# jeff-regier/Celeste.jl

Measured on AMD Instinct MI355X. Metric: sources/sec (ELBO value+gradient+Hessian+KL per target source), higher is better.
Workload: dtype f64; 1 GPU; BASELINE.json configs[2]: synthetic 2048x1489x5 SDSS-size field, 2000 star+galaxy sources, fp64, Sa=1 with value-only neighbours, psf_K=2; gather_backend=none, neighbor_links_rank0=3526

## Files before the change

### celeste.jl_amd/csrc/celeste_abi.hip

```cpp
#include <hip/hip_runtime.h>
#include <algorithm>
#include <atomic>
#include <cmath>
#include <cstdio>
#include <cstdlib>
#include <cstring>
#include <mutex>
#include <unordered_map>
#include <vector>

#include "elbo_kernels.h"
#include "optim_kernels.h"
#include "fused_kernels.h"
#include "host_tables.h"
#include "value_union.h"

struct celeste_group;

#define EVAL_FUSED_MAX 32

#define HIP_TRY(expr)                                                                    \
    do {                                                                                 \
        hipError_t e__ = (expr);                                                         \
        if (e__ != hipSuccess) {                                                         \
// ... 87 lines not shown
    std::vector<void *> plane_allocs;
    DevImage *d_images = nullptr;
    std::atomic<int> refs{1};
};

static void images_release(celeste_images *im) {
    if (!im || im->refs.fetch_sub(1) != 1) return;
    (void)hipSetDevice(im->device);
    for (void *p : im->plane_allocs) (void)hipFree(p);
    if (im->d_images) (void)hipFree(im->d_images);
    delete im;
}

struct celeste_ctx {
    int device = 0;
    celeste_images *imgs = nullptr;
    hipStream_t stream = nullptr;
    hipStream_t copy_stream = nullptr;
    bool copy_stream_checked = false;
    int N = 0, S = 0, K = 0, NC = 0, n_stamps = 0;
    int chunk_px = 256, CH = 1;
    int max_npx = 0;
    std::vector<DevPatch> h_patches;
    std::vector<int64_t> h_nbr_off;
    std::vector<int32_t> h_nbr_idx;
    DevImage *d_images = nullptr;
    DevPatch *d_patches = nullptr;
    double *d_coefs = nullptr;
    float *d_coefs_f = nullptr;
    uint8_t *d_bitmaps = nullptr;
    int64_t *d_nbr_off = nullptr;
    int32_t *d_nbr_idx = nullptr;
    PriorDev *d_prior = nullptr;
    SrcImg *d_srcimg = nullptr;
    Comp *d_comps = nullptr;
    SrcGeo *d_geo = nullptr;
    int64_t *d_val_off = nullptr;
    double2 *d_val = nullptr;
    int32_t *d_needed = nullptr;
    int32_t stamp = 0;
    std::vector<int32_t> h_vis_off, h_vis_img, h_vis_src;
    int32_t *d_vis_off = nullptr, *d_vis_img = nullptr, *d_vis_src = nullptr;
    int4 *d_value_items = nullptr;
    int4 *d_vitems_src = nullptr;
    int32_t *d_vitem_off = nullptr;
    std::vector<int32_t> h_vitem_off;
    std::vector<int32_t> h_vitem_tgt;
    std::vector<ValueUnionLink> h_vitem_link;
    int64_t n_value_items = 0;
    std::vector<struct celeste_targets *> lists;
    int32_t *d_prep_mark = nullptr;
    double *d_lg_sum = nullptr;
    int64_t *d_nv_base = nullptr;
    int32_t *d_nbr_vis = nullptr;
    int2 *d_items = nullptr;
    size_t items_cap = 0;
    std::vector<int32_t> h_src_chunks;
    std::vector<int64_t> h_top_chunks;
    int max_src_chunks = 0;
    int32_t *d_work = nullptr, *d_work_blk = nullptr, *d_work_total = nullptr;
    size_t work_cap = 0, work_blk_cap = 0;
    int M = 1;
    bool dense = false;
    int64_t V = 0;
    std::vector<int64_t> h_tile_off;
    int64_t *d_tile_off = nullptr;
    int64_t n_tiles = 0;
    int sum_tiles = 4, RCH = 1;
    double *d_rec = nullptr;
    double *d_acc_split = nullptr;
    size_t acc_split_cap = 0;
    double *d_acc = nullptr;
    size_t acc_cap = 0;
    int32_t *d_rec_off = nullptr;
    size_t rec_off_cap = 0;
    double *d_vp = nullptr;
    int32_t *d_targets = nullptr;
    double *d_v = nullptr, *d_d = nullptr, *d_h = nullptr;
    int64_t *d_cnt = nullptr;
    int32_t *d_status = nullptr;
    size_t stage_cap = 0;
    double *p_vp = nullptr;
    int32_t *p_targets = nullptr, *p_status = nullptr;
    double *p_v = nullptr, *p_d = nullptr, *p_h = nullptr;
    int64_t *p_cnt = nullptr;
    size_t pin_cap = 0;
    double *d_small_in = nullptr, *p_small_in = nullptr, *d_small_out = nullptr, *p_small_out = nullptr;
    static const int MAX_PARTS = 8;
    hipEvent_t part_done[MAX_PARTS] = {}, part_copied[MAX_PARTS] = {};
    struct OptBuffers {
        size_t cap = 0;
        double *d_vp = nullptr, *d_v = nullptr, *d_d = nullptr, *d_h = nullptr, *d_H = nullptr, *d_T = nullptr, *d_S = nullptr, *d_pos = nullptr;
        int32_t *d_targets = nullptr, *d_act[2] = {nullptr, nullptr}, *d_evt[2] = {nullptr, nullptr}, *d_count = nullptr,
                *d_st = nullptr;
        void *d_state = nullptr;
        static const int RING = 4;
        double *h_vp = nullptr;
        void *h_state = nullptr;
        int32_t *h_count = nullptr;
        hipEvent_t ev[RING] = {};
    } opt;
    struct FusedBuffers {
        size_t cap_t = 0, cap_rec = 0, cap_q = 0, cap_saved = 0;
        bool arrivals_dirty = true;
        int4 *d_chunk_desc = nullptr;
        int2 *d_tgt_rec = nullptr;
// ... 294 lines not shown
            if (device >= 0 && device < 16) consts_ready[device] = true;
        }
    }
    CTX_TRY(dev_upload<SrcImg>(&c->d_srcimg, nullptr, (size_t)c->V));
    CTX_TRY(dev_upload<Comp>(&c->d_comps, nullptr, (size_t)c->V * c->NC));
    CTX_TRY(dev_upload<SrcGeo>(&c->d_geo, nullptr, (size_t)c->S));
    {
        std::vector<int64_t> voff(c->h_patches.size());
        int64_t tot = 0;
        for (size_t q = 0; q < c->h_patches.size(); ++q) { voff[q] = tot; tot += (int64_t)c->h_patches[q].H2 * c->h_patches[q].W2; }
        CTX_TRY(dev_upload(&c->d_val_off, voff.data(), voff.size()));
        CTX_TRY(dev_upload<double2>(&c->d_val, nullptr, (size_t)tot));
        CTX_TRY(dev_upload<int32_t>(&c->d_needed, nullptr, (size_t)c->S));
        if (hipMemset(c->d_needed, 0, (size_t)c->S * sizeof(int32_t)) != hipSuccess) { celeste_ctx_destroy(c); return CELESTE_ERR_HIP; }
    }

    CTX_TRY(dev_upload(&c->d_vis_off, c->h_vis_off.data(), c->h_vis_off.size()));
    CTX_TRY(dev_upload(&c->d_vis_img, c->h_vis_img.data(), c->h_vis_img.size()));
    CTX_TRY(dev_upload(&c->d_vis_src, c->h_vis_src.data(), c->h_vis_src.size()));
    CTX_TRY(dev_upload<double>(&c->d_lg_sum, nullptr, (size_t)c->V));
    if (c->V > 0)
        hipLaunchKernelGGL(patch_lgamma_kernel, dim3((unsigned)c->V), dim3(256), 0, nullptr, c->d_images, c->d_patches,
                           c->d_vis_img, c->d_bitmaps, c->d_lg_sum);
    const char *env_chunk = getenv("CELESTE_CHUNK_PX");
    if (env_chunk && atoi(env_chunk) >= 64) c->chunk_px = (atoi(env_chunk) + 63) / 64 * 64;
    c->CH = c->max_npx > 0 ? (c->max_npx + c->chunk_px - 1) / c->chunk_px : 1;
    c->h_src_chunks.assign((size_t)c->S, 0);
    for (int s = 0; s < c->S; ++s) {
        for (int v = c->h_vis_off[s]; v < c->h_vis_off[s + 1]; ++v) {
            const DevPatch &q = c->h_patches[v];
            c->h_src_chunks[s] += (q.H2 * q.W2 + c->chunk_px - 1) / c->chunk_px;
        }
        c->max_src_chunks = std::max(c->max_src_chunks, c->h_src_chunks[s]);
    }
    auto hv = [c](int s, int n) -> int64_t {
        if (c->dense) return (int64_t)s * c->N + n;
        const int32_t *b = c->h_vis_img.data() + c->h_vis_off[s], *e = c->h_vis_img.data() + c->h_vis_off[s + 1];
        const int32_t *it = std::lower_bound(b, e, n);
        return it != e && *it == n ? (int64_t)(it - c->h_vis_img.data()) : -1;
    };
    if (!c->dense) {
        std::vector<int64_t> base((size_t)c->S + 1, 0);
        for (int s = 0; s < c->S; ++s)
            base[s + 1] = base[s] + (int64_t)(c->h_vis_off[s + 1] - c->h_vis_off[s]) * (c->h_nbr_off[s + 1] - c->h_nbr_off[s]);
        std::vector<int32_t> nv((size_t)base[c->S]);
        for (int s = 0; s < c->S; ++s) {
            const int64_t K = c->h_nbr_off[s + 1] - c->h_nbr_off[s];
            for (int v = c->h_vis_off[s]; v < c->h_vis_off[s + 1]; ++v)
                for (int64_t q = 0; q < K; ++q)
                    nv[base[s] + (int64_t)(v - c->h_vis_off[s]) * K + q] = (int32_t)hv(c->h_nbr_idx[c->h_nbr_off[s] + q], c->h_vis_img[v]);
        }
        CTX_TRY(dev_upload(&c->d_nv_base, base.data(), base.size()));
        CTX_TRY(dev_upload(&c->d_nbr_vis, nv.data(), nv.size()));
    }
    {
        std::vector<int32_t> sorted(c->h_src_chunks);
        std::sort(sorted.begin(), sorted.end(), [](int32_t a, int32_t b) { return a > b; });
        c->h_top_chunks.assign((size_t)c->S + 1, 0);
        for (int s = 0; s < c->S; ++s) c->h_top_chunks[s + 1] = c->h_top_chunks[s] + sorted[s];
    }
    CTX_TRY(dev_upload<int32_t>(&c->d_work_total, nullptr, 1));
    {
        if (c->N > 0xffff) { celeste_ctx_destroy(c); return CELESTE_ERR_INVALID_ARG; }
        const int n_cls = c->chunk_px / 64;
        std::vector<std::vector<std::pair<int32_t, int32_t>>> by_len(n_cls);
        for (int s = 0; s < c->S; ++s)
            for (int64_t q = c->h_nbr_off[s]; q < c->h_nbr_off[s + 1]; ++q) {
                const int s2 = c->h_nbr_idx[q];
                for (int va = c->h_vis_off[s]; va < c->h_vis_off[s + 1]; ++va) {
                    const int n = c->h_vis_img[va];
                    const int64_t vb = hv(s2, n);
                    if (vb < 0) continue;
                    const DevPatch &a = c->h_patches[va], &b = c->h_patches[vb];
                    const int rh = std::min(a.off_h + a.H2, b.off_h + b.H2) - std::max(a.off_h, b.off_h);
                    const int rw = std::min(a.off_w + a.W2, b.off_w + b.W2 - 1) - std::max(a.off_w, b.off_w);
                    if (rh <= 0 || rw <= 0) continue;
                    const int npx = rh * rw, nch = (npx + c->chunk_px - 1) / c->chunk_px;
                    for (int ch = 0; ch < nch; ++ch) {
                        const int px = std::min(c->chunk_px, npx - ch * c->chunk_px);
                        by_len[n_cls - (px + 63) / 64].push_back({(int32_t)q, (int32_t)(n | (ch << 16))});
                    }
                }
            }
        std::vector<int32_t> link_src(c->h_nbr_idx.size());
        for (int s = 0; s < c->S; ++s)
            for (int64_t q = c->h_nbr_off[s]; q < c->h_nbr_off[s + 1]; ++q) link_src[q] = s;
        std::vector<int4> desc;
        for (auto &v : by_len)
            for (auto &e : v) {
                const int t = link_src[e.first], s2 = c->h_nbr_idx[e.first], n = e.second & 0xffff, ch = e.second >> 16;
                desc.push_back(make_int4((int)hv(s2, n), (int)hv(t, n), ch, t));
            }
        c->n_value_items = (int64_t)desc.size();
        c->h_vitem_tgt.resize(desc.size());
        c->h_vitem_link.resize(desc.size());
        for (size_t i = 0; i < desc.size(); ++i) { c->h_vitem_tgt[i] = desc[i].w; c->h_vitem_link[i] = {desc[i].x, desc[i].y}; }
        CTX_TRY(dev_upload(&c->d_value_items, desc.data(), desc.size()));
        c->h_vitem_off.assign((size_t)c->S + 1, 0);
        for (auto &d : desc) c->h_vitem_off[(size_t)d.w + 1]++;
        for (int s = 0; s < c->S; ++s) c->h_vitem_off[s + 1] += c->h_vitem_off[s];
        {
            std::vector<int4> by_src(desc.size());
            std::vector<int32_t> fill(c->h_vitem_off.begin(), c->h_vitem_off.end() - 1);
            for (auto &d : desc) by_src[(size_t)fill[d.w]++] = d;
            CTX_TRY(dev_upload(&c->d_vitems_src, by_src.data(), by_src.size()));
            CTX_TRY(dev_upload(&c->d_vitem_off, c->h_vitem_off.data(), c->h_vitem_off.size()));
// ... 312 lines not shown
        if (flags & CELESTE_FLAG_HESS) LAUNCH_PIXEL_M(2);
        else if (derivs) LAUNCH_PIXEL_M(1);
        else LAUNCH_PIXEL_M(0);
    }
    else if (split) LAUNCH_PIXEL(3);
    else if (flags & CELESTE_FLAG_HESS) LAUNCH_PIXEL(2);
    else if (derivs) LAUNCH_PIXEL(1);
    else LAUNCH_PIXEL_T(0, double);
#undef LAUNCH_PIXEL
#undef LAUNCH_PIXEL_M
#undef PIXEL_ARGS
#undef LAUNCH_PIXEL_T
    if (c->timing) HIP_TRY(hipEventRecord(c->ev[2], stream));
    c->ev_split = 0;
    const int lift_nt = n_targets <= 1024 ? 512 : 256;
    bool lift7 = n_targets > 4096;
    if (const char *e = getenv("CELESTE_LIFT_WAVES")) lift7 = atoi(e) == 7;
#define LAUNCH_LIFT(...) do { if (lift7) hipLaunchKernelGGL(lift_kernel<7>, __VA_ARGS__); else hipLaunchKernelGGL(lift_kernel<8>, __VA_ARGS__); } while (0)
    if (split) {
        hipLaunchKernelGGL(record_sum_kernel, dim3((unsigned)((size_t)n_targets * c->M * c->RCH)), dim3(RSUM_NT), 0,
                           stream, c->d_patches, d_targets, c->d_tile_off, reinterpret_cast<const double2 *>(c->d_rec),
                           c->d_items, c->N, c->M, c->RCH, c->sum_tiles, c->d_acc_split, nullptr, c->d_work_total);
        if (c->timing) { HIP_TRY(hipEventRecord(c->ev[4], stream)); c->ev_split = 1; }
        LAUNCH_LIFT(dim3(n_targets), dim3(lift_nt), 0, stream, d_vp, c->d_images, c->d_patches, c->d_geo,
                           c->d_nbr_off, c->d_nbr_idx, d_targets, c->d_acc_split, c->d_prior, c->d_vis_off, c->d_vis_img, c->N, c->M,
                           c->RCH, c->sum_tiles * 64, flags,
                           d_v, d_d, d_h, d_counters, d_status, d_live, d_active_rank ? nullptr : c->d_lg_sum, nullptr, d_h_pos);
    } else
    LAUNCH_LIFT(dim3(n_targets), dim3(lift_nt), 0, stream, d_vp, c->d_images, c->d_patches, c->d_geo,
                       c->d_nbr_off, c->d_nbr_idx, d_targets, c->d_acc, c->d_prior, c->d_vis_off, c->d_vis_img, c->N, c->M, CH,
                       chunk_px, flags,
                       d_v, d_d, d_h, d_counters, d_status, d_live, d_active_rank ? nullptr : c->d_lg_sum, c->d_rec_off, d_h_pos);
#undef LAUNCH_LIFT
    if (c->timing) { HIP_TRY(hipEventRecord(c->ev[3], stream)); c->ev_valid = 1; }
    HIP_TRY(hipGetLastError());
    return CELESTE_OK;
}

struct celeste_targets {
    celeste_ctx_t *ctx = nullptr;
    int32_t n = 0;
    int G = 1;
    int32_t *d_targets = nullptr;
    int32_t *d_work = nullptr, *d_work_total = nullptr, *d_rec_off = nullptr;
    int2 *d_items = nullptr;
    int32_t *d_needed = nullptr;
    int32_t *d_visits = nullptr;
    int32_t *d_vitems = nullptr;
    int4 *d_uitems = nullptr;
    int32_t *d_upx = nullptr;
    int64_t n_visits = 0, n_vitems = 0, n_uitems = 0;
    int64_t n_records = 0;
    int32_t n_work = 0;
};
static const int32_t LIST_STAMP = 1;

static void targets_free(celeste_targets *t) {
    if (!t) return;
    void *ptrs[] = {t->d_targets, t->d_work, t->d_work_total, t->d_rec_off, t->d_items, t->d_needed, t->d_visits, t->d_vitems,
                    t->d_uitems, t->d_upx};
    for (void *p : ptrs) if (p) (void)hipFree(p);
    delete t;
}

static int targets_build(celeste_ctx_t *c, const std::vector<int32_t> &tg, celeste_targets_t **out) {
    const int32_t n = (int32_t)tg.size();
    if ((size_t)n * c->M * c->CH > 0x7fffffffull) return CELESTE_ERR_INVALID_ARG;
    HIP_TRY(hipSetDevice(c->device));
    celeste_targets *t = new celeste_targets;
    t->ctx = c; t->n = n; t->G = chunk_group(n);
    int32_t *d_blk = nullptr;
    auto fail = [&](int st) { if (d_blk) (void)hipFree(d_blk); (void)hipGetLastError(); targets_free(t); return st; };
#define LIST_TRY(expr) do { if ((expr) != hipSuccess) return fail(CELESTE_ERR_HIP); } while (0)
#define LIST_ALLOC(p, bytes) do { if (hipMalloc((void **)&(p), (bytes)) != hipSuccess) return fail(CELESTE_ERR_ALLOC); } while (0)
    std::vector<char> is_tgt((size_t)c->S, 0), reads((size_t)c->S, 0);
    for (int32_t s : tg) {
        is_tgt[s] = 1; reads[s] = 1;
        for (int64_t q = c->h_nbr_off[s]; q < c->h_nbr_off[s + 1]; ++q) reads[c->h_nbr_idx[q]] = 1;
        t->n_records += c->h_src_chunks[s];
    }
    std::vector<int32_t> visits, vitems;
    for (int s = 0; s < c->S; ++s)
        if (reads[s]) for (int v = c->h_vis_off[s]; v < c->h_vis_off[s + 1]; ++v) visits.push_back(v);
    for (size_t i = 0; i < c->h_vitem_tgt.size(); ++i) if (is_tgt[c->h_vitem_tgt[i]]) vitems.push_back((int32_t)i);
    std::vector<int32_t> upx;
    std::vector<ValueUnionItem> uitems;
    {
        static_assert(sizeof(ValueUnionBox) == 4 * sizeof(int32_t) && sizeof(ValueUnionItem) == sizeof(int4), "layout");
        std::vector<ValueUnionBox> boxes(c->h_patches.size());
        for (size_t v = 0; v < boxes.size(); ++v) { const DevPatch &q = c->h_patches[v]; boxes[v] = {q.off_h, q.off_w, q.H2, q.W2}; }
        std::vector<ValueUnionLink> links;
        links.reserve(vitems.size());
        for (int32_t i : vitems) links.push_back(c->h_vitem_link[(size_t)i]);
        if (!value_union_build(boxes.data(), std::move(links), c->chunk_px, upx, uitems)) return fail(CELESTE_ERR_INVALID_ARG);
    }
    t->n_visits = (int64_t)visits.size(); t->n_vitems = (int64_t)vitems.size(); t->n_uitems = (int64_t)uitems.size();
    const int n_cand = n * c->M;
    const int n_wblk = (n_cand + WORK_NT - 1) / WORK_NT;
    const size_t n_blk = (size_t)n_wblk * (WORK_CLASSES + 1);
    LIST_ALLOC(t->d_targets, (size_t)n * sizeof(int32_t));
    LIST_ALLOC(t->d_work, std::max<size_t>((size_t)t->n_records, 1) * sizeof(int32_t));
    LIST_ALLOC(t->d_work_total, sizeof(int32_t));
    LIST_ALLOC(t->d_rec_off, (size_t)n_cand * sizeof(int32_t));
    if (!c->dense) LIST_ALLOC(t->d_items, (size_t)n_cand * sizeof(int2));
    LIST_ALLOC(t->d_needed, (size_t)c->S * sizeof(int32_t));
    LIST_ALLOC(t->d_visits, std::max<size_t>(visits.size(), 1) * sizeof(int32_t));
    LIST_ALLOC(t->d_vitems, std::max<size_t>(vitems.size(), 1) * sizeof(int32_t));
    LIST_ALLOC(t->d_uitems, std::max<size_t>(uitems.size(), 1) * sizeof(int4));
    LIST_ALLOC(t->d_upx, std::max<size_t>(upx.size(), 1) * sizeof(int32_t));
    LIST_ALLOC(d_blk, n_blk * sizeof(int32_t));
    LIST_TRY(hipMemcpy(t->d_targets, tg.data(), (size_t)n * sizeof(int32_t), hipMemcpyHostToDevice));
    if (!visits.empty()) LIST_TRY(hipMemcpy(t->d_visits, visits.data(), visits.size() * sizeof(int32_t), hipMemcpyHostToDevice));
    if (!vitems.empty()) LIST_TRY(hipMemcpy(t->d_vitems, vitems.data(), vitems.size() * sizeof(int32_t), hipMemcpyHostToDevice));
    if (!uitems.empty()) LIST_TRY(hipMemcpy(t->d_uitems, uitems.data(), uitems.size() * sizeof(int4), hipMemcpyHostToDevice));
    if (!upx.empty()) LIST_TRY(hipMemcpy(t->d_upx, upx.data(), upx.size() * sizeof(int32_t), hipMemcpyHostToDevice));
    LIST_TRY(hipMemset(t->d_needed, 0, (size_t)c->S * sizeof(int32_t)));
    const size_t setup_threads = (size_t)n * (c->dense ? 1 : c->M);
    hipLaunchKernelGGL(setup_kernel, dim3((unsigned)((setup_threads + 63) / 64)), dim3(64), 0, nullptr, (const double *)nullptr, -1,
                       (SrcGeo *)nullptr, t->d_targets, n, c->d_vis_off, c->d_vis_img, c->M, t->d_items, t->d_needed, LIST_STAMP,
                       (int32_t *)nullptr, c->d_nbr_off, c->d_nbr_idx, (const int32_t *)nullptr);
    hipLaunchKernelGGL(work_count_kernel, dim3(n_wblk), dim3(WORK_NT), 0, nullptr, t->d_targets, n_cand, c->d_patches,
                       c->d_vis_off, c->d_vis_img, c->N, c->M, c->chunk_px, t->G, (int)c->dense, d_blk, (const int32_t *)nullptr);
    hipLaunchKernelGGL(work_scan_kernel, dim3(1), dim3(1024), 0, nullptr, d_blk, (int)n_blk, t->d_work_total, n_wblk * WORK_CLASSES);
    hipLaunchKernelGGL(work_fill_kernel, dim3(n_wblk), dim3(WORK_NT), 0, nullptr, t->d_targets, n_cand, c->d_patches,
                       c->d_vis_off, c->d_vis_img, c->N, c->M, c->CH, c->chunk_px, t->G, (int)c->dense, d_blk, t->d_work,
                       (const int32_t *)nullptr, t->d_rec_off);
    LIST_TRY(hipGetLastError());
    LIST_TRY(hipMemcpy(&t->n_work, t->d_work_total, sizeof(int32_t), hipMemcpyDeviceToHost));
    LIST_TRY(hipFree(d_blk)); d_blk = nullptr;
#undef LIST_TRY
#undef LIST_ALLOC
    if (t->n_work < 0 || (int64_t)t->n_work > t->n_records) return fail(CELESTE_ERR_HIP);
    c->lists.push_back(t);
    *out = t;
    return CELESTE_OK;
}

extern "C" int celeste_targets_create(celeste_ctx_t *c, int32_t n_targets, const int32_t *targets, celeste_targets_t **out) try {
    if (!c || !out || !targets || n_targets <= 0) return CELESTE_ERR_INVALID_ARG;
    *out = nullptr;
    for (int32_t i = 0; i < n_targets; ++i) if (targets[i] < 0 || targets[i] >= c->S) return CELESTE_ERR_INVALID_ARG;
    return targets_build(c, std::vector<int32_t>(targets, targets + n_targets), out);
} ABI_CATCH

extern "C" int celeste_targets_create_device(celeste_ctx_t *c, int32_t n_targets, const int32_t *d_targets, void *stream_,
                                             celeste_targets_t **out) try {
    if (!c || !out || !d_targets || n_targets <= 0) return CELESTE_ERR_INVALID_ARG;
    *out = nullptr;
    HIP_TRY(hipSetDevice(c->device));
    std::vector<int32_t> tg((size_t)n_targets);
    HIP_TRY(hipMemcpyAsync(tg.data(), d_targets, (size_t)n_targets * sizeof(int32_t), hipMemcpyDeviceToHost, (hipStream_t)stream_));
    HIP_TRY(hipStreamSynchronize((hipStream_t)stream_));
    for (int32_t s : tg) if (s < 0 || s >= c->S) return CELESTE_ERR_INVALID_ARG;
    return targets_build(c, tg, out);
} ABI_CATCH

static void targets_release(celeste_targets_t *t) {
    celeste_ctx_t *c = t->ctx;
    auto it = std::find(c->lists.begin(), c->lists.end(), t);
    if (it != c->lists.end()) c->lists.erase(it);
    targets_free(t);
}

extern "C" void celeste_targets_destroy(celeste_targets_t *t) {
    if (!t) return;
    (void)hipSetDevice(t->ctx->device);
    (void)hipDeviceSynchronize();
    targets_release(t);
}

static int launch_prepared(celeste_ctx_t *c, const celeste_targets_t *t, const double *d_vp, uint32_t flags, double *d_v,
                           double *d_d, double *d_h, int64_t *d_counters, int32_t *d_status, void *stream_) {
    if (!c || !t || t->ctx != c) return CELESTE_ERR_INVALID_ARG;
    const int32_t n_targets = t->n;
    const char *off = getenv("CELESTE_NO_PREPARED");
    if ((off && atoi(off) != 0) || (flags & (CELESTE_FLAG_FP32 | CELESTE_FLAG_SPLIT)) ||
        want_eval_fused(flags, n_targets, true, d_d, d_h))
        return launch_eval(c, d_vp, n_targets, t->d_targets, flags, d_v, d_d, d_h, d_counters, d_status, stream_, true, nullptr,
                           t->n_records);
    if (!d_vp || !d_v || !d_status) return CELESTE_ERR_INVALID_ARG;
    if ((flags & CELESTE_FLAG_HESS) && !d_h) return CELESTE_ERR_INVALID_ARG;
    if ((flags & (CELESTE_FLAG_GRAD | CELESTE_FLAG_HESS)) && !d_d) return CELESTE_ERR_INVALID_ARG;
    hipStream_t stream = (hipStream_t)stream_;
    HIP_TRY(hipSetDevice(c->device));
    const size_t need = std::max<size_t>((size_t)t->n_records, 1) * ACC_N;
    if (need > c->acc_cap) {
        if (c->d_acc) { HIP_TRY(hipStreamSynchronize(stream)); HIP_TRY(hipFree(c->d_acc)); c->d_acc = nullptr; }
        HIP_TRY(hipMalloc((void **)&c->d_acc, need * sizeof(double)));
        c->acc_cap = need;
    }
    const int CH = c->CH, chunk_px = c->chunk_px;
    if (c->timing) HIP_TRY(hipEventRecord(c->ev[0], stream));
    const unsigned geo_blocks = (unsigned)((c->S + 63) / 64);
    hipLaunchKernelGGL(geo_prep_kernel, dim3(geo_blocks + (unsigned)t->n_visits), dim3(64), 0, stream, d_vp, c->d_images,
                       c->d_patches, c->d_vis_src, c->d_vis_img, c->K, c->d_srcimg, c->d_comps, t->d_visits, (int)geo_blocks,
                       c->S, c->d_geo);
    const char *no_union = getenv("CELESTE_NO_VALUE_UNION");
    if (!(no_union && atoi(no_union) != 0)) {
        if (t->n_uitems > 0) {
            const bool wide_items = n_targets <= VALUE_WIDE_MAX && c->chunk_px == 256 && !getenv("CELESTE_NO_WIDE_VALUE");
#define LAUNCH_UNION(WAVES)                                                                                                 \
            hipLaunchKernelGGL((value_union_kernel<WAVES>), dim3((unsigned)t->n_uitems), dim3(64 * WAVES), 0, stream,       \
                               c->d_patches, c->d_coefs, c->d_srcimg, c->d_comps, c->d_val_off, t->d_uitems, t->d_upx,      \
                               c->NC, c->d_val)
            if (wide_items) LAUNCH_UNION(4); else LAUNCH_UNION(1);
#undef LAUNCH_UNION
        }
    } else if (t->n_vitems > 0) {
        const bool wide_items = n_targets <= VALUE_WIDE_MAX && c->chunk_px == 256 && !getenv("CELESTE_NO_WIDE_VALUE");
#define LAUNCH_VALUE(WAVES)                                                                                                 \
        hipLaunchKernelGGL((value_kernel<double, WAVES>), dim3((unsigned)t->n_vitems), dim3(64 * WAVES), 0, stream,        \
                           c->d_patches, c->d_coefs, c->d_srcimg, c->d_comps, t->d_needed, LIST_STAMP, c->d_val_off,        \
                           c->d_value_items, c->NC, c->chunk_px, c->d_val, c->d_coefs_f, t->d_vitems)
        if (wide_items) LAUNCH_VALUE(4); else LAUNCH_VALUE(1);
#undef LAUNCH_VALUE
    }
    if (c->timing) HIP_TRY(hipEventRecord(c->ev[1], stream));
    const dim3 grid((unsigned)std::max<int32_t>(t->n_work, 1));
#define LAUNCH_PIXEL(MODE)                                                                                                  \
    hipLaunchKernelGGL((pixel_kernel<MODE, double>), grid, dim3(64), 0, stream, c->d_images, c->d_patches, c->d_coefs,      \
                       c->d_bitmaps, c->d_srcimg, c->d_comps, c->d_nbr_off, c->d_nbr_idx, c->d_val_off, c->d_val,           \
                       t->d_targets, c->N, c->NC, CH, chunk_px, t->G, c->d_acc, c->d_tile_off, c->d_rec,                    \
                       (const int32_t *)nullptr, t->d_items, c->M, t->d_work, t->d_work_total, c->d_nv_base, c->d_nbr_vis,  \
                       t->d_rec_off, c->d_coefs_f)
    if (flags & CELESTE_FLAG_HESS) LAUNCH_PIXEL(2);
    else if (flags & CELESTE_FLAG_GRAD) LAUNCH_PIXEL(1);
    else LAUNCH_PIXEL(0);
#undef LAUNCH_PIXEL
    if (c->timing) HIP_TRY(hipEventRecord(c->ev[2], stream));
    c->ev_split = 0;
    const int lift_nt = n_targets <= 1024 ? 512 : 256;
    bool lift7 = n_targets > 4096;
    if (const char *e = getenv("CELESTE_LIFT_WAVES")) lift7 = atoi(e) == 7;
#define LIFT_ARGS dim3(n_targets), dim3(lift_nt), 0, stream, d_vp, c->d_images, c->d_patches, c->d_geo, c->d_nbr_off,       \
                  c->d_nbr_idx, t->d_targets, c->d_acc, c->d_prior, c->d_vis_off, c->d_vis_img, c->N, c->M, CH, chunk_px,   \
                  flags, d_v, d_d, d_h, d_counters, d_status, (const int32_t *)nullptr, c->d_lg_sum, t->d_rec_off, \
                  (const int32_t *)nullptr
    if (lift7) hipLaunchKernelGGL(lift_kernel<7>, LIFT_ARGS); else hipLaunchKernelGGL(lift_kernel<8>, LIFT_ARGS);
#undef LIFT_ARGS
    if (c->timing) { HIP_TRY(hipEventRecord(c->ev[3], stream)); c->ev_valid = 1; }
    HIP_TRY(hipGetLastError());
    return CELESTE_OK;
}

extern "C" int celeste_elbo_eval_targets_device(celeste_ctx_t *c, const celeste_targets_t *t, const double *d_vp, uint32_t flags,
                                                double *d_v, double *d_d, double *d_h, int64_t *d_counters,
                                                int32_t *d_status, void *stream_) try {
    return launch_prepared(c, t, d_vp, flags, d_v, d_d, d_h, d_counters, d_status, stream_);
} ABI_CATCH

__global__ void spin_kernel(long long ticks) {
    const long long t0 = wall_clock64();
    while (wall_clock64() - t0 < ticks) __builtin_amdgcn_s_sleep(8);
}
static int pick_copy_stream(celeste_ctx_t *c) {
    if (c->copy_stream_checked) return CELESTE_OK;
    c->copy_stream_checked = true;
    if (const char *e = getenv("CELESTE_COPY_STREAM_CHECK")) if (atoi(e) == 0) return CELESTE_OK;
    const size_t bytes = 4u << 20;
    void *d_buf = nullptr, *h_buf = nullptr;
    hipEvent_t e0 = nullptr, e1 = nullptr;
    if (hipMalloc(&d_buf, bytes) != hipSuccess || hipHostMalloc(&h_buf, bytes, hipHostMallocDefault) != hipSuccess ||
        hipEventCreate(&e0) != hipSuccess || hipEventCreate(&e1) != hipSuccess) {
        (void)hipGetLastError();
        if (d_buf) (void)hipFree(d_buf);
        if (h_buf) (void)hipHostFree(h_buf);
        if (e0) (void)hipEventDestroy(e0);
        if (e1) (void)hipEventDestroy(e1);
        return CELESTE_OK;
    }
    const float spin_ms = 0.3f;
    auto measure = [&](hipStream_t s, float *ms) -> bool {
        if (hipEventRecord(e0, c->stream) != hipSuccess) return false;
        hipLaunchKernelGGL(spin_kernel, dim3(1), dim3(64), 0, c->stream, (long long)(spin_ms * 1e5));
        if (hipStreamWaitEvent(s, e0, 0) != hipSuccess || hipMemcpyAsync(h_buf, d_buf, bytes, hipMemcpyDeviceToHost, s) != hipSuccess ||
            hipEventRecord(e1, s) != hipSuccess || hipStreamSynchronize(s) != hipSuccess || hipStreamSynchronize(c->stream) != hipSuccess)
            return false;
        return hipEventElapsedTime(ms, e0, e1) == hipSuccess;
// ... 1016 lines not shown
```

### celeste.jl_amd/csrc/elbo_kernels.h

```cpp
#pragma once
#include <hip/hip_runtime.h>
#include <math.h>
#include "elbo_device.h"
#include "../../include/celeste_mi355x.h"

#ifndef CELESTE_MUTANT
#define CELESTE_MUTANT 0
#endif

__constant__ double c_eta[16];
__constant__ double c_nu[16];

__device__ inline void bvn_cov(double ab, double angle, double scale, double &x11, double &x12, double &x22) {
    double sp, cp;
    sincos(angle, &sp, &cp);
    double ab_term = ab * ab - 1.0;
    double s2 = scale * scale;
    x12 = -s2 * cp * sp * ab_term;
    x11 = s2 * (1.0 + ab_term * (sp * sp));
    x22 = s2 * (1.0 + ab_term * (cp * cp));
}

__device__ inline void brightness(const double *vs, int i, int b, double &El, double &Ell) {
    const double r = vs[6 + i], v = vs[8 + i];
    const double *cm = vs + 10 + 4 * i, *cv = vs + 18 + 4 * i;
    double l = r + 0.5 * v, ll = 2 * r + 2 * v;
    if (b >= 3) { l += cm[2] + .5 * cv[2]; ll += 2 * cm[2] + 2 * cv[2]; }
    if (b >= 4) { l += cm[3] + .5 * cv[3]; ll += 2 * cm[3] + 2 * cv[3]; }
    if (b <= 1) { l += -cm[1] + .5 * cv[1]; ll += -2 * cm[1] + 2 * cv[1]; }
    if (b <= 0) { l += -cm[0] + .5 * cv[0]; ll += -2 * cm[0] + 2 * cv[0]; }
    double e = exp(r + 0.5 * v), ee = exp(2 * r + 2 * v);
    if (b >= 3) { e *= exp(cm[2] + .5 * cv[2]); ee *= exp(2 * cm[2] + 2 * cv[2]); }
    if (b >= 4) { e *= exp(cm[3] + .5 * cv[3]); ee *= exp(2 * cm[3] + 2 * cv[3]); }
    if (b <= 1) { e *= exp(-cm[1] + .5 * cv[1]); ee *= exp(-2 * cm[1] + 2 * cv[1]); }
    if (b <= 0) { e *= exp(-cm[0] + .5 * cv[0]); ee *= exp(-2 * cm[0] + 2 * cv[0]); }
    (void)l; (void)ll;
    El = e; Ell = ee;
}

__device__ __forceinline__ void world_to_pix(const double *__restrict__ vs, const DevPatch &p, double &m1, double &m2) {
    const double d0 = vs[0] - p.wc[0], d1 = vs[1] - p.wc[1];
    m1 = p.J[0] * d0 + p.J[2] * d1 + p.pc[0];
    m2 = p.J[1] * d0 + p.J[3] * d1 + p.pc[1];
}
template <bool MOMENTS = true>
__device__ __forceinline__ void prep_visit_values(int c, const double *__restrict__ vs, const DevPatch &p, int b, int K,
                                                  SrcImg *__restrict__ si_out, Comp *__restrict__ comps_out) {
    const int NC = 14 * K;
    double m1, m2;
    world_to_pix(vs, p, m1, m2);
    double x11, x12, x22;
    bvn_cov(vs[3], vs[4], vs[5], x11, x12, x22);
    if (c < NC) {
        int i, j, k;
        if (c < 8 * K) { i = 0; k = c / 8; j = c - 8 * k; }
        else { int cc = c - 8 * K; i = 1; k = cc / 6; j = cc - 6 * k; }
// ... 1913 lines not shown
        __syncthreads();
    }
    __shared__ double tcx[(MODE == 2 || MODE == 3) && sizeof(R) == 8 ? COMPX * (14 * CEL_MAXK + 1) : 1];
    if constexpr ((MODE == 2 || MODE == 3) && sizeof(R) == 8) {
        if (lane < NC) comp_extra(tc[lane], tcx + COMPX * lane);
        __syncthreads();
    }
    PixWork<R> W;
    W.img = &images[n]; W.P = &P; W.patches = patches; W.bitmaps = bitmaps; W.nbr_idx = nbr_idx;
    W.nb0 = nbr_off[t]; W.nb1 = nbr_off[t + 1];
    W.nv = nbr_vis ? nbr_vis + nv_base[t] + (int64_t)(tn - ti * M) * (W.nb1 - W.nb0) : nullptr;
    W.val_off = val_off; W.val = val; W.active_rank = active_rank;
    W.my_rank = MULTI ? active_rank[t] : 0;
    W.N = N; W.n = n; W.NC = NC; W.v = v;
    W.si = srcimg[v];
    W.tc = tc; W.tcx = tcx;
    W.tcr = sizeof(R) == 4 ? reinterpret_cast<const CompR<R> *>(tcr_f) : reinterpret_cast<const CompR<R> *>(tc);
    W.etab = etab;
    W.tcoef = coefs + (size_t)(CELESTE_MUTANT == 3 ? 0 : P.stamp) * (CEL_COEF * CEL_COEF);
    W.tcoef_f = coefs_f + (size_t)(CELESTE_MUTANT == 3 ? 0 : P.stamp) * (CEL_COEF * CEL_COEF);
    W.tile_off = tile_off; W.rec = rec;
    __shared__ double sacc[MODE == 0 || MODE == 3 ? 1 : ACC_N * ACC_SLOTS];
    double *const slot = sacc + (lane & (ACC_SLOTS - 1));
    for (int ch = ch0; ch < ch0 + G && ch * chunk_px < npx; ++ch) {
    const int p0 = ch * chunk_px;
    const int p1 = min(npx, p0 + chunk_px);
    const int wg = rec_base + ch;
    if constexpr (MODE == 1 || MODE == 2) {
#pragma unroll
        for (int i = 0; i < ACC_N * ACC_SLOTS / 64; ++i) sacc[lane + 64 * i] = 0.0;
        __syncthreads();
    }
    double a[3] = {0.0, 0.0, 0.0};

    if constexpr (sizeof(R) == 4 && (MODE == 1 || MODE == 2) && !MULTI) {
        for (int base = p0; base < p1; base += 128) pixel_iter_px2<MODE>(W, base, p1, lane, slot);
    } else
    for (int base = p0; base < p1; base += 64) pixel_iter<MODE, R, MULTI>(W, base, p1, lane, slot, a, []() {});
    if (MODE == 3) continue;

    double *__restrict__ out = acc + (size_t)wg * ACC_N;
    if (MODE == 0) {
        const double s0 = wave_sum(a[0]), s1 = wave_sum(a[1]), s2 = wave_sum(a[2]);
        if (lane == 0) { out[0] = s0; out[ACC_CNT] = s1; out[ACC_CNT + 1] = s2; }
        continue;
    }
    __syncthreads();
    fold_record_slots<MODE>(sacc, lane, [&](int e, double s) { out[e] = s; });
    __syncthreads();
    }
    }
}

typedef double d2v __attribute__((ext_vector_type(2)));
#define RSUM_NT 128
#define RSUM_K (ACC_N * 32 / RSUM_NT)
__global__ void __launch_bounds__(RSUM_NT)
record_sum_kernel(const DevPatch *__restrict__ patches, const int32_t *__restrict__ targets,
                  const int64_t *__restrict__ tile_off, const double2 *__restrict__ rec,
                  const int2 *__restrict__ items, int N, int M, int RCH, int sum_tiles,
                  double *__restrict__ acc, const int32_t *__restrict__ work, const int32_t *__restrict__ work_total) {
    int part, tn;
    if (work) {
        if ((int)blockIdx.x >= *work_total) return;
        const int wg = work[blockIdx.x];
        tn = wg / RCH; part = wg - tn * RCH;
    } else {
        const int TN = gridDim.x / RCH;
        part = blockIdx.x / TN;
        tn = blockIdx.x - part * TN;
    }
    const int ti = tn / M;
    const int t = targets[ti];
    const int vis = items ? items[tn].x : t * N + (tn - ti * M);
    if (vis < 0) return;
    const DevPatch &P = patches[vis];
    const int npx = P.H2 * P.W2;
    const int tile0 = part * sum_tiles;
    const int ntiles = min(sum_tiles, ((npx + 63) >> 6) - tile0);
    if (ntiles <= 0) return;
    const int tid = threadIdx.x;
    const d2v *__restrict__ src = reinterpret_cast<const d2v *>(rec) +
                                  (size_t)(tile_off[vis] + tile0) * (ACC_N * 32) + tid;
    d2v a[RSUM_K];
#pragma unroll
    for (int k = 0; k < RSUM_K; ++k) a[k] = (d2v)(0.0);
    for (int tile = 0; tile < ntiles; ++tile) {
        d2v v[RSUM_K];
#pragma unroll
        for (int k = 0; k < RSUM_K; ++k) v[k] = __builtin_nontemporal_load(src + k * RSUM_NT);
#pragma unroll
        for (int k = 0; k < RSUM_K; ++k) a[k] += v[k];
        src += ACC_N * 32;
    }
    double *__restrict__ out = acc + ((size_t)tn * RCH + part) * ACC_N;
    const int row0 = tid >> 5;
#pragma unroll
    for (int k = 0; k < RSUM_K; ++k) {
        double s = a[k].x + a[k].y;
        s += __shfl_xor(s, 16); s += __shfl_xor(s, 8); s += __shfl_xor(s, 4); s += __shfl_xor(s, 2); s += __shfl_xor(s, 1);
        if ((tid & 31) == 0) out[row0 + 4 * k] = s;
    }
}

struct PriorDev {
    celeste_prior_t p;
// ... 810 lines not shown
```

Measured before the change: 3.221 million sources/sec.

## Precompute per-work-item descriptors on host and launch descriptor-driven pixel kernel

At target-list build time, the host now reads back the work list and record offsets and builds a compact 64-byte descriptor per work item. Each descriptor holds the patch geometry, neighbour range, nbr_vis row, image index and record base. Descriptors are sorted by descending trip count, so long items start first. A new pixel_desc_kernel reads one descriptor per block instead of decoding the work id and chasing the patch, offset and visibility tables, and it drops the multi-rank and tiled paths. This aims to cut per-block setup indirection and tail imbalance, at the cost of extra host work and device-to-host copies during list setup.

```diff
diff --git a/celeste.jl_amd/csrc/celeste_abi.hip b/celeste.jl_amd/csrc/celeste_abi.hip
--- a/celeste.jl_amd/csrc/celeste_abi.hip
+++ b/celeste.jl_amd/csrc/celeste_abi.hip
@@ -163,6 +163,7 @@
     int32_t *d_prep_mark = nullptr;
     double *d_lg_sum = nullptr;
     int64_t *d_nv_base = nullptr;
+    std::vector<int64_t> h_nv_base;
     int32_t *d_nbr_vis = nullptr;
     int2 *d_items = nullptr;
     size_t items_cap = 0;
@@ -563,6 +564,7 @@
         }
         CTX_TRY(dev_upload(&c->d_nv_base, base.data(), base.size()));
         CTX_TRY(dev_upload(&c->d_nbr_vis, nv.data(), nv.size()));
+        c->h_nv_base.swap(base);
     }
     {
         std::vector<int32_t> sorted(c->h_src_chunks);
@@ -981,13 +983,15 @@
     int64_t n_visits = 0, n_vitems = 0, n_uitems = 0;
     int64_t n_records = 0;
     int32_t n_work = 0;
+    WorkSeqDesc *d_desc = nullptr;
+    int32_t n_desc = 0;
 };
 static const int32_t LIST_STAMP = 1;
 
 static void targets_free(celeste_targets *t) {
     if (!t) return;
     void *ptrs[] = {t->d_targets, t->d_work, t->d_work_total, t->d_rec_off, t->d_items, t->d_needed, t->d_visits, t->d_vitems,
-                    t->d_uitems, t->d_upx};
+                    t->d_uitems, t->d_upx, t->d_desc};
     for (void *p : ptrs) if (p) (void)hipFree(p);
     delete t;
 }
@@ -1057,9 +1061,39 @@
     LIST_TRY(hipGetLastError());
     LIST_TRY(hipMemcpy(&t->n_work, t->d_work_total, sizeof(int32_t), hipMemcpyDeviceToHost));
     LIST_TRY(hipFree(d_blk)); d_blk = nullptr;
+    if (t->n_work < 0 || (int64_t)t->n_work > t->n_records) return fail(CELESTE_ERR_HIP);
+    {
+        std::vector<int32_t> h_work((size_t)t->n_work), h_rec_off((size_t)n_cand);
+        if (t->n_work > 0) LIST_TRY(hipMemcpy(h_work.data(), t->d_work, h_work.size() * sizeof(int32_t), hipMemcpyDeviceToHost));
+        if (n_cand > 0) LIST_TRY(hipMemcpy(h_rec_off.data(), t->d_rec_off, h_rec_off.size() * sizeof(int32_t), hipMemcpyDeviceToHost));
+        std::vector<WorkSeqDesc> items;
+        std::vector<int32_t> trips, order;
+        items.reserve(h_work.size()); trips.reserve(h_work.size());
+        for (int32_t wg0 : h_work) {
+            if (wg0 < 0 || wg0 / c->CH >= n_cand) return fail(CELESTE_ERR_HIP);
+            const int tn = wg0 / c->CH, ch0 = wg0 - tn * c->CH, ti = tn / c->M, j = tn - ti * c->M, s = tg[(size_t)ti];
+            if (j >= c->h_vis_off[s + 1] - c->h_vis_off[s]) continue;
+            const int32_t v = c->h_vis_off[s] + j;
+            const DevPatch &q = c->h_patches[(size_t)v];
+            const int n_trips = work_item_trips(q.H2 > 0 && q.W2 > 0 ? (int64_t)q.H2 * q.W2 : 0, ch0, t->G, c->chunk_px);
+            if (n_trips <= 0) continue;
+            const int64_t nbn = c->h_nbr_off[s + 1] - c->h_nbr_off[s];
+            if (nbn > 0x7fffffffll) return fail(CELESTE_ERR_INVALID_ARG);
+            WorkSeqDesc D{};
+            D.off_h = q.off_h; D.off_w = q.off_w; D.H2 = q.H2; D.W2 = q.W2; D.bitmap_off = q.bitmap_off; D.stamp = q.stamp;
+            D.nb0 = c->h_nbr_off[s]; D.nbn = (int32_t)nbn; D.nv_row = c->dense ? 0 : c->h_nv_base[s] + (int64_t)j * nbn;
+            D.v = v; D.n = c->h_vis_img[(size_t)v]; D.rec_base = h_rec_off[(size_t)tn]; D.ch0 = ch0;
+            order.push_back((int32_t)items.size()); items.push_back(D); trips.push_back(n_trips);
+        }
+        std::stable_sort(order.begin(), order.end(), [&](int32_t a, int32_t b) { return trips[(size_t)a] > trips[(size_t)b]; });
+        std::vector<WorkSeqDesc> sorted(items.size());
+        for (size_t i = 0; i < order.size(); ++i) sorted[i] = items[(size_t)order[i]];
+        t->n_desc = (int32_t)sorted.size();
+        LIST_ALLOC(t->d_desc, std::max<size_t>(sorted.size(), 1) * sizeof(WorkSeqDesc));
+        if (!sorted.empty()) LIST_TRY(hipMemcpy(t->d_desc, sorted.data(), sorted.size() * sizeof(WorkSeqDesc), hipMemcpyHostToDevice));
+    }
 #undef LIST_TRY
 #undef LIST_ALLOC
-    if (t->n_work < 0 || (int64_t)t->n_work > t->n_records) return fail(CELESTE_ERR_HIP);
     c->lists.push_back(t);
     *out = t;
     return CELESTE_OK;
@@ -1145,14 +1179,26 @@
 #undef LAUNCH_VALUE
     }
     if (c->timing) HIP_TRY(hipEventRecord(c->ev[1], stream));
-    const dim3 grid((unsigned)std::max<int32_t>(t->n_work, 1));
+    const char *no_seq = getenv("CELESTE_NO_SEQUENCES");
+    const bool sequences = !(no_seq && atoi(no_seq) != 0);
+    const dim3 grid((unsigned)std::max<int32_t>(sequences ? t->n_desc : t->n_work, 1));
+#define LAUNCH_SEQ(MODE)                                                                                                    \
+    hipLaunchKernelGGL((pixel_desc_kernel<MODE>), grid, dim3(64), 0, stream, c->d_images, c->d_patches, c->d_coefs,         \
+                       c->d_bitmaps, c->d_srcimg, c->d_comps, c->d_nbr_idx, c->d_val_off, c->d_val, c->N, c->NC, chunk_px,  \
+                       t->G, c->d_acc, t->d_desc, t->n_desc, c->d_nbr_vis, c->d_coefs_f)
+    if (!sequences) { }
+    else if (flags & CELESTE_FLAG_HESS) LAUNCH_SEQ(2);
+    else if (flags & CELESTE_FLAG_GRAD) LAUNCH_SEQ(1);
+    else LAUNCH_SEQ(0);
+#undef LAUNCH_SEQ
 #define LAUNCH_PIXEL(MODE)                                                                                                  \
     hipLaunchKernelGGL((pixel_kernel<MODE, double>), grid, dim3(64), 0, stream, c->d_images, c->d_patches, c->d_coefs,      \
                        c->d_bitmaps, c->d_srcimg, c->d_comps, c->d_nbr_off, c->d_nbr_idx, c->d_val_off, c->d_val,           \
                        t->d_targets, c->N, c->NC, CH, chunk_px, t->G, c->d_acc, c->d_tile_off, c->d_rec,                    \
                        (const int32_t *)nullptr, t->d_items, c->M, t->d_work, t->d_work_total, c->d_nv_base, c->d_nbr_vis,  \
                        t->d_rec_off, c->d_coefs_f)
-    if (flags & CELESTE_FLAG_HESS) LAUNCH_PIXEL(2);
+    if (sequences) { }
+    else if (flags & CELESTE_FLAG_HESS) LAUNCH_PIXEL(2);
     else if (flags & CELESTE_FLAG_GRAD) LAUNCH_PIXEL(1);
     else LAUNCH_PIXEL(0);
 #undef LAUNCH_PIXEL
diff --git a/celeste.jl_amd/csrc/elbo_kernels.h b/celeste.jl_amd/csrc/elbo_kernels.h
--- a/celeste.jl_amd/csrc/elbo_kernels.h
+++ b/celeste.jl_amd/csrc/elbo_kernels.h
@@ -2,6 +2,7 @@
 #include <hip/hip_runtime.h>
 #include <math.h>
 #include "elbo_device.h"
+#include "work_sequences.h"
 #include "../../include/celeste_mi355x.h"
 
 #ifndef CELESTE_MUTANT
@@ -2021,6 +2022,96 @@
     }
 }
 
+template <int MODE>
+__global__ void __launch_bounds__(64, PIXEL_WAVES)
+pixel_desc_kernel(const DevImage *__restrict__ images, const DevPatch *__restrict__ patches,
+                  const double *__restrict__ coefs, const uint8_t *__restrict__ bitmaps,
+                  const SrcImg *__restrict__ srcimg, const Comp *__restrict__ comps,
+                  const int32_t *__restrict__ nbr_idx, const int64_t *__restrict__ val_off, const double2 *__restrict__ val,
+                  int N, int NC, int chunk_px, int G, double *__restrict__ acc,
+                  const WorkSeqDesc *__restrict__ desc, int n_items,
+                  const int32_t *__restrict__ nbr_vis, const float *__restrict__ coefs_f) {
+    static_assert(MODE == 0 || MODE == 1 || MODE == 2, "the prepared path: value, gradient, Hessian");
+    static_assert(offsetof(DevPatch, off_h) == offsetof(WorkSeqDesc, off_h) && offsetof(DevPatch, off_w) == offsetof(WorkSeqDesc, off_w) &&
+                  offsetof(DevPatch, H2) == offsetof(WorkSeqDesc, H2) && offsetof(DevPatch, W2) == offsetof(WorkSeqDesc, W2) &&
+                  offsetof(DevPatch, bitmap_off) == offsetof(WorkSeqDesc, bitmap_off) &&
+                  offsetof(DevPatch, stamp) == offsetof(WorkSeqDesc, stamp), "the descriptor's head is DevPatch's");
+    if ((int)blockIdx.x >= n_items) return;
+    __shared__ double etab[64];
+    __shared__ Comp tc[14 * CEL_MAXK + 1];
+    __shared__ double tcx[MODE == 2 ? COMPX * (14 * CEL_MAXK + 1) : 1];
+    __shared__ double sacc[MODE == 0 ? 1 : ACC_N * ACC_SLOTS];
+    const int lane = threadIdx.x;
+    double *const slot = sacc + (lane & (ACC_SLOTS - 1));
+    const WorkSeqDesc &D = desc[blockIdx.x];
+    const int v = D.v;
+    const SrcImg si = srcimg[v];
+    {
+        constexpr int ROUNDS = (14 * CEL_MAXK * 8 + 63) / 64;
+        const double *src = reinterpret_cast<const double *>(comps + (size_t)v * NC);
+        double *dst = reinterpret_cast<double *>(tc);
+        const double tabv = g_exp2_table[lane];
+        Comp own;
+        if constexpr (MODE == 2) {
+            const Comp &k = comps[(size_t)v * NC + min(lane, NC - 1)];
+            own.p11 = k.p11; own.p12 = k.p12; own.p22 = k.p22;
+        }
+        double r[ROUNDS];
+#pragma unroll
+        for (int k = 0; k < ROUNDS; ++k) r[k] = src[min(lane + 64 * k, NC * 8 - 1)];
+        if constexpr (MODE == 1 || MODE == 2) {
+#pragma unroll
+            for (int i = 0; i < ACC_N * ACC_SLOTS / 64; ++i) sacc[lane + 64 * i] = 0.0;
+        }
+        etab[lane] = tabv;
+#pragma unroll
+        for (int k = 0; k < ROUNDS; ++k) if (lane + 64 * k < NC * 8) dst[lane + 64 * k] = r[k];
+        if constexpr (MODE == 2) {
+            if (lane < NC) comp_extra(own, tcx + COMPX * lane);
+        }
+        __syncthreads();
+    }
+    PixWork<double> W;
+    W.img = &images[D.n]; W.P = reinterpret_cast<const DevPatch *>(&D); W.patches = patches; W.bitmaps = bitmaps; W.nbr_idx = nbr_idx;
+    W.nb0 = D.nb0; W.nb1 = D.nb0 + D.nbn;
+    W.nv = nbr_vis ? nbr_vis + D.nv_row : nullptr;
+    W.val_off = val_off; W.val = val; W.active_rank = nullptr;
+    W.my_rank = 0;
+    W.N = N; W.n = D.n; W.NC = NC; W.v = v;
+    W.si = si;
+    W.tc = tc; W.tcx = tcx;
+    W.tcr = reinterpret_cast<const CompR<double> *>(tc);
+    W.etab = etab;
+    W.tcoef = coefs + (size_t)(CELESTE_MUTANT == 3 ? 0 : D.stamp) * (CEL_COEF * CEL_COEF);
+    W.tcoef_f = coefs_f + (size_t)(CELESTE_MUTANT == 3 ? 0 : D.stamp) * (CEL_COEF * CEL_COEF);
+    W.tile_off = nullptr; W.rec = nullptr;
+    const int npx = D.H2 * D.W2;
+    const int ch0 = D.ch0;
+    for (int ch = ch0; ch < ch0 + G && ch * chunk_px < npx; ++ch) {
+    const int p0 = ch * chunk_px;
+    const int p1 = min(npx, p0 + chunk_px);
+    const int wg = D.rec_base + ch;
+    if constexpr (MODE == 1 || MODE == 2) {
+        if (ch != ch0) {
+#pragma unroll
+            for (int i = 0; i < ACC_N * ACC_SLOTS / 64; ++i) sacc[lane + 64 * i] = 0.0;
+            __syncthreads();
+        }
+    }
+    double a[3] = {0.0, 0.0, 0.0};
+    for (int base = p0; base < p1; base += 64) pixel_iter<MODE, double, false>(W, base, p1, lane, slot, a, []() {});
+    double *__restrict__ out = acc + (size_t)wg * ACC_N;
+    if (MODE == 0) {
+        const double s0 = wave_sum(a[0]), s1 = wave_sum(a[1]), s2 = wave_sum(a[2]);
+        if (lane == 0) { out[0] = s0; out[ACC_CNT] = s1; out[ACC_CNT + 1] = s2; }
+        continue;
+    }
+    __syncthreads();
+    fold_record_slots<MODE>(sacc, lane, [&](int e, double s) { out[e] = s; });
+    __syncthreads();
+    }
+}
+
 typedef double d2v __attribute__((ext_vector_type(2)));
 #define RSUM_NT 128
 #define RSUM_K (ACC_N * 32 / RSUM_NT)
diff --git a/celeste.jl_amd/csrc/work_sequences.h b/celeste.jl_amd/csrc/work_sequences.h
--- /dev/null
+++ b/celeste.jl_amd/csrc/work_sequences.h
@@ -0,0 +1,26 @@
+#pragma once
+#include <cstddef>
+#include <cstdint>
+
+struct alignas(64) WorkSeqDesc {
+    int32_t off_h, off_w, H2, W2;
+    int64_t bitmap_off;
+    int32_t stamp;
+    int32_t nbn;
+    int64_t nb0;
+    int64_t nv_row;
+    int32_t v, n;
+    int32_t rec_base;
+    int32_t ch0;
+};
+static_assert(sizeof(WorkSeqDesc) == 64 && offsetof(WorkSeqDesc, bitmap_off) == 16 && offsetof(WorkSeqDesc, stamp) == 24,
+              "one uniform 64-byte load per item");
+
+inline int work_item_trips(int64_t npx, int ch0, int G, int chunk_px) {
+    int trips = 0;
+    for (int ch = ch0; ch < ch0 + G && (int64_t)ch * chunk_px < npx; ++ch) {
+        const int64_t p0 = (int64_t)ch * chunk_px, p1 = npx < p0 + chunk_px ? npx : p0 + chunk_px;
+        trips += (int)((p1 - p0 + 63) / 64);
+    }
+    return trips;
+}
```

Result: faster. 3.293 million sources/sec (median of 6 runs) (+2.2%).
